# lmdu/pyfastx

Measured on AMD Instinct MI355X. Metric: FASTA index build + 1M random 100bp subseq fetches, 3 Gbp plain FASTA per GPU (throughput of the whole step, stream resident in HBM), higher is better.
Workload: dtype u8; 1 GPU; configs[1]: synthetic 3.0 Gbp hg38-shaped plain FASTA per GPU (200 contigs, 60-col LF, soft-masked, N runs), index build + 1000000 random 100 bp intervals (50% '-' strand); parallelism=one GPU, the whole stream resident in its HBM

## Files before the change

pyfastx_amd/csrc/fx_spanscan.hpp:

```cpp
#pragma once
#include "fx_kernels.hpp"

namespace fx {

#ifndef FX_GRAN
#define FX_GRAN 4096
#endif
constexpr int GRAN = FX_GRAN;
constexpr int GR_ROWS = GRAN / (64 * CHUNK);
constexpr int SPAN_GRANS = 65536 / GRAN;
constexpr int SPAN = GRAN * SPAN_GRANS;
constexpr uint32_t SP_NONE = 0xFFFFFFFFu;

struct GranOut { uint32_t n, h, first, last, v1, c1, v2, c2, ovf; };
struct __attribute__((aligned(16))) GranPk { uint32_t nh, fl, d1, d2; };
__device__ __forceinline__ GranPk gran_pack(const GranOut &o) {
    GranPk p;
    p.nh = o.n | (o.h << 16); p.fl = (o.first & 0xFFFFu) | (o.last << 16);
    p.d1 = o.v1 | (o.c1 << 16); p.d2 = o.v2 | (o.c2 << 16) | (o.ovf << 31);
    return p;
}
__device__ __forceinline__ GranOut gran_unpack(const GranPk &p) {
    GranOut o;
    o.n = p.nh & 0xFFFFu; o.h = p.nh >> 16;
// ... 196 lines not shown
#define FX_SCAN_GPW 1
#endif
constexpr int SCAN_GPW = FX_SCAN_GPW;
template <int MODE>
__global__ __launch_bounds__(1024) void k_span_scan(const uint8_t *__restrict__ data, int64_t n, int prev_byte,
                                                   int is_last, int64_t g_end, GranPk *__restrict__ out, GranList hgl) {
    __shared__ uint32_t hl_n, hl_done, hl_g[16 * SCAN_GPW];
    if (MODE == 0) {
        if (threadIdx.x == 0) { hl_n = 0; hl_done = 0; }
        __syncthreads();
    }
    const int64_t g0 = (((int64_t)blockIdx.x * blockDim.x + threadIdx.x) >> 6) * SCAN_GPW;
    uint4 v[SCAN_GPW][GR_ROWS];
#pragma unroll
    for (int k = 0; k < SCAN_GPW; ++k) if (g0 + k < g_end) granule_load<true>(v[k], data, n, is_last, g0 + k);
    uint32_t L = 0, hmask = 0;
#pragma unroll
    for (int k = 0; k < SCAN_GPW; ++k)
        if (g0 + k < g_end && granule_body<MODE>(v[k], data, prev_byte, g0 + k, out, L)) hmask |= 1u << k;
    if (MODE == 0 && lane_id() == 0) {
#pragma unroll
        for (int k = 0; k < SCAN_GPW; ++k) if ((hmask >> k) & 1u) hl_g[atomicAdd(&hl_n, 1u)] = (uint32_t)(g0 + k);
        __threadfence_block();
        if (atomicAdd(&hl_done, 1u) == (blockDim.x >> 6) - 1) {
            const uint32_t cnt = hl_n;
            if (cnt) {
                const uint32_t base = atomicAdd(hgl.count, cnt);
                for (uint32_t k = 0; k < cnt; ++k) hgl.g[base + k] = hl_g[k];
            }
        }
    }
}

constexpr int CHUNK_GRANS = 1024;
struct ChunkTot { long long n, h, last, pad; };
struct Totals {
    long long n_nl, n_hdr, last_nl, seq_len, pad0, pad1, pad2, pad3;
};

__device__ __forceinline__ long long shfl_up64(long long v, int d) {
    const int lo = __shfl_up((int)(v & 0xFFFFFFFFll), d, 64), hi = __shfl_up((int)(v >> 32), d, 64);
    return ((long long)hi << 32) | (unsigned int)lo;
}
__device__ __forceinline__ long long shfl64(long long v, int l) {
    const int lo = __shfl((int)(v & 0xFFFFFFFFll), l, 64), hi = __shfl((int)(v >> 32), l, 64);
    return ((long long)hi << 32) | (unsigned int)lo;
}
struct Tri { long long n, h, last; };
__device__ __forceinline__ Tri tri_join(const Tri &a, const Tri &b) { return Tri{a.n + b.n, a.h + b.h, a.last > b.last ? a.last : b.last}; }
__device__ __forceinline__ Tri tri_wave_incl(Tri v) {
    const int l = lane_id();
#pragma unroll
    for (int d = 1; d < 64; d <<= 1) {
        const Tri t{shfl_up64(v.n, d), shfl_up64(v.h, d), shfl_up64(v.last, d)};
        if (l >= d) v = tri_join(t, v);
    }
    return v;
}
__device__ __forceinline__ Tri tri_block_incl(Tri v, Tri *lds, Tri *total) {
    const int w = threadIdx.x >> 6, l = lane_id(), nw = (blockDim.x + 63) >> 6;
    const Tri inc = tri_wave_incl(v);
    __syncthreads();
    if (l == 63) lds[w] = inc;
    __syncthreads();
    Tri base{0, 0, -1}, tot{0, 0, -1};
    for (int i = 0; i < nw; ++i) { const Tri s = lds[i]; if (i < w) base = tri_join(base, s); tot = tri_join(tot, s); }
    *total = tot;
    return tri_join(base, inc);
}
__device__ __forceinline__ Tri gran_tri(const GranPk *__restrict__ go, int64_t g, int64_t ngran, int64_t gbase) {
    if (g >= ngran) return Tri{0, 0, -1};
    const GranOut o = gran_unpack(go[g]);
    return Tri{(long long)o.n, (long long)o.h, o.n ? gbase + g * (long long)GRAN + o.last : -1};
}

template <int MODE, int CG>
__global__ __launch_bounds__(CG) void k_gran_reduce(const uint8_t *__restrict__ data, int64_t n, int prev_byte,
                                                   int is_last, GranList hgl, GranPk *__restrict__ go,
                                                   int64_t ngran, int64_t gbase, ChunkTot *__restrict__ ct) {
    __shared__ Tri lds[CG / 64];
    if (blockIdx.x == gridDim.x - 1) {
        if (threadIdx.x < 64) {
            uint32_t L = 0;
            const uint32_t h_w = granule<false, MODE>(data, n, prev_byte, is_last, ngran - 1, go, L);
            if (MODE == 0 && h_w && threadIdx.x == 0) hgl.g[atomicAdd(hgl.count, 1u)] = (uint32_t)(ngran - 1);
        }
        __threadfence_block();
        __syncthreads();
    }
    Tri tot;
    tri_block_incl(gran_tri(go, (int64_t)blockIdx.x * CG + threadIdx.x, ngran, gbase), lds, &tot);
    if (threadIdx.x == 0) ct[blockIdx.x] = ChunkTot{tot.n, tot.h, tot.last, 0};
}

struct Tri32 { uint32_t n, h; int32_t last; };
__device__ __forceinline__ Tri32 tri32_block_incl(Tri32 v, uint32_t (*lds)[16], Tri32 *total) {
    const int w = threadIdx.x >> 6, l = lane_id(), nw = (blockDim.x + 63) >> 6;
#pragma unroll
    for (int d = 1; d < 64; d <<= 1) {
        const uint32_t a = __shfl_up(v.n, d, 64), b = __shfl_up(v.h, d, 64);
        const int32_t c = __shfl_up(v.last, d, 64);
        if (l >= d) { v.n += a; v.h += b; v.last = c > v.last ? c : v.last; }
    }
    __syncthreads();
    if (l == 63) { lds[0][w] = v.n; lds[1][w] = v.h; lds[2][w] = (uint32_t)v.last; }
    __syncthreads();
    Tri32 base{0, 0, -1}, tot{0, 0, -1};
    for (int i = 0; i < nw; ++i) {
        const uint32_t a = lds[0][i], b = lds[1][i];
        const int32_t c = (int32_t)lds[2][i];
        if (i < w) { base.n += a; base.h += b; base.last = c > base.last ? c : base.last; }
        tot.n += a; tot.h += b; tot.last = c > tot.last ? c : tot.last;
    }
    *total = tot;
    return Tri32{base.n + v.n, base.h + v.h, base.last > v.last ? base.last : v.last};
}

template <int CG>
__global__ __launch_bounds__(CG) void k_gran_prefix(const GranPk *__restrict__ go, int64_t ngran, int64_t gbase,
                                                            const ChunkTot *__restrict__ ct, Totals *__restrict__ tot,
                                                            int64_t *__restrict__ nl_prefix, int64_t *__restrict__ hdr_prefix,
                                                            int64_t *__restrict__ prevnl) {
    __shared__ Tri lds[CG / 64];
    __shared__ uint32_t lds32[3][16];
    Tri b{0, 0, -1};
    for (int64_t c = threadIdx.x; c < (int64_t)blockIdx.x; c += CG) { const ChunkTot t = ct[c]; b = tri_join(b, Tri{t.n, t.h, t.last}); }
    Tri base{0, 0, -1};
    if (blockIdx.x) tri_block_incl(b, lds, &base);
    const int64_t g = (int64_t)blockIdx.x * CG + threadIdx.x;
    Tri32 v{0, 0, -1};
    if (g < ngran) {
        const GranOut o = gran_unpack(go[g]);
        v = Tri32{o.n, o.h, o.n ? (int32_t)(threadIdx.x * GRAN + o.last) : -1};
    }
    Tri32 total;
    const Tri32 inc = tri32_block_incl(v, lds32, &total);
    const int64_t cstart = gbase + (int64_t)blockIdx.x * CG * GRAN;
    if (g < ngran) {
        nl_prefix[g] = base.n + (inc.n - v.n);
        hdr_prefix[g] = base.h + (inc.h - v.h);
        int32_t pm = __shfl_up(inc.last, 1, 64);
        if (lane_id() == 0) { pm = -1; for (int i = 0; i < (int)(threadIdx.x >> 6); ++i) { const int32_t c = (int32_t)lds32[2][i]; pm = c > pm ? c : pm; } }
        prevnl[g] = pm >= 0 ? cstart + pm : base.last;
    }
    if (blockIdx.x == gridDim.x - 1 && threadIdx.x == 0) {
        const int64_t tn = base.n + total.n, th = base.h + total.h, tl = total.last >= 0 ? cstart + total.last : base.last;
        nl_prefix[ngran] = tn; hdr_prefix[ngran] = th; prevnl[ngran] = tl;
        tot->n_nl = tn; tot->n_hdr = th; tot->last_nl = tl;
    }
}

struct ScanCtx {
    const uint8_t *data; int64_t n, gbase, ngran;
    const GranPk *go;
    const int64_t *nl_prefix, *hdr_prefix, *prevnl;
};

__device__ __forceinline__ int64_t next_nl(const ScanCtx &c, int64_t x) {
    const int64_t y = x + 1 - c.gbase;
    if (y > c.n) return -1;
    const int64_t g = y / GRAN;
    if (g < c.ngran) {
        const GranOut o = gran_unpack(c.go[g]);
        const int64_t gs = g * (int64_t)GRAN;
        if (o.n && gs + o.last >= y) {
            if (gs + o.first >= y) return c.gbase + gs + o.first;
            for (int64_t p = y & ~(int64_t)(CHUNK - 1); p < gs + GRAN; p += CHUNK) {
                const uint4 v = load16(c.data, p, c.n);
                uint32_t m = eq_mask16(v, 0x0A0A0A0Au);
                if (p < y) m &= 0xFFFFu << (y - p);
                if (m) return c.gbase + p + (__ffs(m) - 1);
                if (p + CHUNK > c.n) break;
            }
            return c.gbase + gs + o.last;
        }
    }
    const int64_t key = c.gbase + (g + 1) * (int64_t)GRAN;
    int64_t lo = g + 1, hi = c.ngran;
// ... 285 lines not shown
            return;
        }
    }
    irr.g[atomicAdd(irr.count, 1u)] = (uint32_t)g;
}

__global__ __launch_bounds__(BLOCK) void k_gran_exact(ScanCtx x, RecView rv, int64_t cap, GranList irr, int is_last, int prev_byte) {
    const int lane = lane_id();
    const int64_t wave = ((int64_t)blockIdx.x * blockDim.x + threadIdx.x) >> 6;
    const int64_t nwaves = ((int64_t)gridDim.x * blockDim.x) >> 6;
    const int64_t cnt = *irr.count;
    int64_t i = wave, g = i < cnt ? irr.g[i] : 0;
    uint4 v[GR_ROWS];
    if (i < cnt) {
#pragma unroll
        for (int j = 0; j < GR_ROWS; ++j) v[j] = load16(x.data, g * (int64_t)GRAN + j * 1024 + lane * CHUNK, x.n);
    }
    for (; i < cnt; i += nwaves) {
        const int64_t gc = g, hb = x.hdr_prefix[gc];
        int64_t he = x.hdr_prefix[gc + 1];
        if (he > cap) he = cap;
        ExactMasks mk;
        exact_masks(x, v, is_last, prev_byte, gc, he > hb, mk);
        if (i + nwaves < cnt) {
            g = irr.g[i + nwaves];
#pragma unroll
            for (int j = 0; j < GR_ROWS; ++j) v[j] = load16(x.data, g * (int64_t)GRAN + j * 1024 + lane * CHUNK, x.n);
        }
        exact_rows(x, rv, cap, gc, hb, mk);
    }
}

__global__ __launch_bounds__(BLOCK) void k_fasta_finalize2(int64_t cap, FastaCols c, Totals *__restrict__ tot,
                                                          const uint8_t *__restrict__ data, int64_t n_bytes, int64_t gbase) {
    const int64_t *__restrict__ hdr = c.hoff, *__restrict__ hdr_line = c.hdr_line;
    const int64_t k = (int64_t)blockIdx.x * BLOCK + threadIdx.x;
    const int64_t n_hdr = tot->n_hdr < cap ? tot->n_hdr : cap;
    int64_t s = 0;
    if (k < n_hdr) {
        if (c.dlen[k] >= 0) {
            int64_t hn, Ln;
            if (k + 1 < n_hdr) { hn = hdr[k + 1]; Ln = hdr_line[k + 1]; }
            else               { hn = tot->last_nl + 1; Ln = tot->n_nl; }
            const int64_t nseq = Ln - hdr_line[k] - 1;
            const int64_t blen = hn - c.boff[k];
            s = blen - (int64_t)c.elen[k] * nseq;
            c.blen[k] = blen; c.slen[k] = s;
            const int norm = c.bad[k] > 1 ? 0 : 1;
            c.norm[k] = norm;
            int reg = line_regular(data, n_bytes, gbase, c.boff[k], blen, s, nseq > 0 ? c.llen[k] : 0, c.elen[k], norm);
            if (reg < 0) reg = c.bad[k] == 0;
            c.reg[k] = reg;
        } else { c.blen[k] = 0; c.slen[k] = 0; c.norm[k] = 1; c.reg[k] = 0; }
    }
    __shared__ unsigned long long blk;
    if (threadIdx.x == 0) blk = 0;
    __syncthreads();
    s = wave_sum64(s);
    if (lane_id() == 0 && s) atomicAdd(&blk, (unsigned long long)s);
    __syncthreads();
    if (threadIdx.x == 0 && blk) atomicAdd((unsigned long long *)&tot->seq_len, blk);
}

__global__ __launch_bounds__(BLOCK) void k_line_regular(const uint8_t *__restrict__ data, int64_t n_bytes, int64_t gbase, int64_t n,
                                                       const int64_t *__restrict__ boff, const int64_t *__restrict__ blen,
                                                       const int64_t *__restrict__ slen, const int64_t *__restrict__ llen,
                                                       const int32_t *__restrict__ elen, const int32_t *__restrict__ norm,
                                                       int32_t *__restrict__ reg) {
    const int64_t k = (int64_t)blockIdx.x * BLOCK + threadIdx.x;
    if (k < n) reg[k] = line_regular(data, n_bytes, gbase, boff[k], blen[k], slen[k], llen[k], elen[k], norm[k]) > 0 ? 1 : 0;
}

__device__ __forceinline__ int64_t prev_nl_wave(const ScanCtx &x, int64_t p) {
    const int64_t y = (p - x.gbase < x.n) ? p - x.gbase : x.n;
    if (y <= 0) return -1;
    const int64_t g = (y - 1) / GRAN;
    const int64_t a = g * (int64_t)GRAN + lane_id() * 64;
    unsigned long long m = 0;
#pragma unroll
    for (int i = 0; i < 4; ++i)
        if (a + i * CHUNK < y) m |= (unsigned long long)eq_mask16(load16(x.data, a + i * CHUNK, x.n), 0x0A0A0A0Au) << (16 * i);
    if (y - a < 64) m &= (y - a <= 0) ? 0ull : (~0ull >> (64 - (y - a)));
    const unsigned long long b = __ballot(m != 0);
    if (!b) return x.prevnl[g];
    const int l = 63 - __clzll(b);
    const int hi = __shfl((int)(m >> 32), l, 64), lo = __shfl((int)(m & 0xFFFFFFFFull), l, 64);
    const unsigned long long ml = ((unsigned long long)(unsigned int)hi << 32) | (unsigned int)lo;
    return x.gbase + g * (int64_t)GRAN + l * 64 + (63 - __clzll(ml));
}

constexpr int SUMM_BLOCK = 1024;
__device__ __forceinline__ DiffSet diffset_shfl_xor(const DiffSet &d, int m) {
    return DiffSet{(uint32_t)__shfl_xor((int)d.v1, m, 64), (uint32_t)__shfl_xor((int)d.c1, m, 64), (uint32_t)__shfl_xor((int)d.v2, m, 64),
                   (uint32_t)__shfl_xor((int)d.c2, m, 64), (uint32_t)__shfl_xor((int)d.ovf, m, 64)};
// ... 210 lines not shown
```

pyfastx_amd/csrc/fxgpu.hip:

```cpp
#include <hip/hip_runtime.h>
#include <zlib.h>
#include <fcntl.h>
#include <pthread.h>
#include <sched.h>
#include <sys/mman.h>
#include <sys/stat.h>
#include <unistd.h>

#include <algorithm>
#include <atomic>
#include <chrono>
#include <functional>
#include <map>
#include <memory>
#include <cstdarg>
#include <cstdio>
#include <cstdlib>
#include <cstring>
#include <mutex>
#include <string>
#include <thread>
#include <vector>

#include "../../include/fxgpu.h"
// ... 223 lines not shown
        if (count <= 0) return FX_OK;
        dev = device;
        stream = st;
        p = (T *)g_scratch.get(device, (size_t)count * sizeof(T), &cap_bytes);
        if (!p) return fail(FX_ENOMEM, "hipMalloc(%lld B) failed", (long long)(count * sizeof(T)));
        return FX_OK;
    }
    void release() {
        if (p) { (void)hipStreamSynchronize(stream); g_scratch.put(dev, p, cap_bytes); }
        p = nullptr; cap_bytes = 0;
    }
    ~ScratchBuf() { release(); }
};

static void crc_tables(CrcTables *T) {
    for (uint32_t i = 0; i < 256; ++i) { uint32_t c = i; for (int k = 0; k < 8; ++k) c = (c & 1) ? 0xEDB88320u ^ (c >> 1) : c >> 1; T->crc[0][i] = c; }
    for (int j = 1; j < 4; ++j)
        for (uint32_t i = 0; i < 256; ++i) T->crc[j][i] = (T->crc[j - 1][i] >> 8) ^ T->crc[0][T->crc[j - 1][i] & 0xFFu];
    uint32_t a[32], b[32];
    a[0] = 0xEDB88320u;
    for (int n = 1; n < 32; ++n) a[n] = 1u << (n - 1);
    auto times = [](const uint32_t *mat, uint32_t vec) { uint32_t s = 0; for (int i = 0; vec; vec >>= 1, ++i) if (vec & 1) s ^= mat[i]; return s; };
    for (int r = 0; r < 3; ++r) { for (int n = 0; n < 32; ++n) b[n] = times(a, a[n]); memcpy(a, b, sizeof a); }
    for (int j = 0; j < 17; ++j) {
        memcpy(T->pow2[j], a, sizeof a);
        for (int n = 0; n < 32; ++n) b[n] = times(a, a[n]);
        memcpy(a, b, sizeof a);
    }
    for (int k = 0; k < CRC_NSH; ++k)
        for (int byte = 0; byte < 4; ++byte)
            for (uint32_t v = 0; v < 256; ++v) T->sh[k][byte][v] = times(T->pow2[CRC_SH0 + k], v << (8 * byte));
}

enum KernelId { K_SPAN_SCAN = 0, K_GRAN_REDUCE, K_GRAN_PREFIX, K_HDR_REC, K_GRAN_LINES, K_GRAN_EXACT, K_FASTA_FINALIZE, K_FETCH,
                K_FASTA_COMP, K_FASTA_COMP_EDGE, K_FASTA_COMP_SMALL, K_FASTQ_LINES, K_FASTQ_ROWS, K_FASTQ_EMIT, K_FASTQ_STATS, K_FASTQ_COMP, K_FASTQ_FETCH, K_BGZF_INFLATE, K_BGZF_COPY, K_BGZF_CRC, K_SCAN_COMP, K_COMP_ATTRIBUTE, K_BGZF_SERIAL, K_FETCH_REST, K_KQ_LINES, K_KQ_PREFIX, K_KQ_WALK, K_KQ_GATHER, K_NKERN };
static const char *const kKernelNames[K_NKERN] = {
    "k_span_scan", "k_gran_reduce", "k_gran_prefix", "k_hdr_rec", "k_gran_lines", "k_gran_exact", "k_fasta_finalize", "k_fetch",
    "k_fasta_comp", "k_fasta_comp_edge", "k_fasta_comp_small", "k_fastq_lines", "k_fastq_rows", "k_fastq_emit", "k_fastq_stats", "k_fastq_comp", "k_fastq_fetch", "k_bgzf_decode", "k_bgzf_copy", "k_bgzf_crc", "k_scan_comp", "k_comp_attribute", "k_bgzf_decode_serial", "k_fetch_rest", "k_kq_lines", "k_kq_prefix", "k_kq_walk", "k_kq_gather"};

struct Prof {
    bool on = false;
    uint32_t mask = ~0u;
    struct Span { int id; hipEvent_t a, b; };
    std::vector<Span> pending;
    std::vector<hipEvent_t> pool;
    double ms[K_NKERN] = {0};
    int64_t cnt[K_NKERN] = {0};
    hipEvent_t get() {
        if (!pool.empty()) { hipEvent_t e = pool.back(); pool.pop_back(); return e; }
        hipEvent_t e = nullptr;
        (void)hipEventCreate(&e);
        return e;
    }
    bool hit = false;
    void begin(int id, hipStream_t s) {
        hit = on && ((mask >> id) & 1u);
        if (!hit) return;
        Span sp{id, get(), get()};
        (void)hipEventRecord(sp.a, s);
        pending.push_back(sp);
    }
    void end(hipStream_t s) { if (hit) (void)hipEventRecord(pending.back().b, s); }
    void drain() {
        for (auto &sp : pending) {
            float t = 0.f;
            if (hipEventElapsedTime(&t, sp.a, sp.b) == hipSuccess) { ms[sp.id] += t; cnt[sp.id]++; }
            pool.push_back(sp.a); pool.push_back(sp.b);
        }
        pending.clear();
    }
    ~Prof() { drain(); for (auto e : pool) (void)hipEventDestroy(e); }
};
#define FX_LAUNCH(h, id, kern, grid, block, ...)                                  \
    do {                                                                          \
        (h)->prof.begin(id, (h)->stream);                                         \
        hipLaunchKernelGGL(kern, grid, block, 0, (h)->stream, __VA_ARGS__);       \
        (h)->prof.end((h)->stream);                                               \
    } while (0)

struct StageAsync;
static void stage_drop(fx_handle *h);
struct fx_handle {
    int device = 0;
    hipStream_t stream = nullptr;
    StageAsync *stage = nullptr;
    int stage_fd = -1;
    hipStream_t stream2 = nullptr;
    uint8_t *d_data = nullptr;
    uint8_t *d_alloc = nullptr;
    size_t blob_cap = 0;
    bool owns = false;
    int64_t n = 0;
    bool gz = false;
    int64_t base = 0;
    int prev_byte = '\n';
    bool is_last = true;
    int64_t n_nl = 0;
    bool scanned = false;
    int64_t ngran = 0;
    DevBuf<GranPk> gran;
    DevBuf<uint32_t> hdr_grans, irr_grans;
    DevBuf<ChunkTot> chunks;
    DevBuf<unsigned long long> ctl;
    Totals *pin_tot = nullptr;
    struct OneBox { int64_t off, blen, skip, take, dst_off, out_len; } *one_box = nullptr;
    uint8_t *one_out = nullptr;
    Mailbox *mb = nullptr;
    hipStream_t mb_stream = nullptr;
    unsigned long long mb_seq = 0;
    bool mb_running = false, mb_off = false;
    DevBuf<uint32_t> nm_table;
    DevBuf<int64_t> nm_off;
    uint64_t nm_mask = 0;
    int nm_kind = -1;
    DevBuf<int64_t> nl_prefix, hdr_prefix, prevnl;
    DevBuf<int64_t> hdr, fa_boff, fa_blen, fa_slen, fa_llen, fa_hdr_line;
    DevBuf<int32_t> fa_elen, fa_norm, fa_dlen, fa_name_len, fa_reg;
    DevBuf<uint32_t> fa_bad;
    int64_t n_hdr = 0, fa_seqlen = 0;
    bool fasta_built = false;
    bool build_pending = false;
    int pending_full_name = 0;
    DevBuf<uint32_t> comp_runs;
    int comp_gpw = 0;
    bool comp_runs_valid = false;
    DevBuf<int64_t> fq_name_off, fq_rlen, fq_soff, fq_qoff;
    DevBuf<int32_t> fq_name_len, fq_dlen, fq_qlen;
    DevBuf<FastqAcc> fq_acc;
    DevBuf<FqRun> fq_runs;
    DevBuf<FastqAcc> fq_acc_build;
    DevBuf<uint32_t> fq_rej;
    int64_t fq_comp_runs = 0, fq_comp_rejected = 0;
    bool fq_comp_valid = false;
    int64_t fq_comp_base[5] = {0, 0, 0, 0, 0};
    int fq_comp_minqs = 104, fq_comp_maxqs = 33;
// ... 1530 lines not shown
    ScanCtx x;
    x.data = h->d_data; x.n = h->n; x.gbase = h->base; x.ngran = h->ngran;
    x.go = h->gran.p; x.nl_prefix = h->nl_prefix.p; x.hdr_prefix = h->hdr_prefix.p; x.prevnl = h->prevnl.p;
    return x;
}
static FastaCols fasta_cols(fx_handle *h) {
    FastaCols c;
    c.hoff = h->hdr.p; c.boff = h->fa_boff.p; c.blen = h->fa_blen.p; c.slen = h->fa_slen.p; c.llen = h->fa_llen.p;
    c.hdr_line = h->fa_hdr_line.p; c.elen = h->fa_elen.p; c.dlen = h->fa_dlen.p; c.name_len = h->fa_name_len.p;
    c.norm = h->fa_norm.p; c.bad = h->fa_bad.p; c.reg = h->fa_reg.p;
    return c;
}
static int alloc_fasta_table(fx_handle *h, int64_t cap) {
    int rc;
    if ((rc = h->hdr.alloc(cap)) || (rc = h->fa_hdr_line.alloc(cap)) || (rc = h->fa_boff.alloc(cap)) ||
        (rc = h->fa_blen.alloc(cap)) || (rc = h->fa_slen.alloc(cap)) || (rc = h->fa_llen.alloc(cap)) ||
        (rc = h->fa_elen.alloc(cap)) || (rc = h->fa_norm.alloc(cap)) || (rc = h->fa_dlen.alloc(cap)) ||
        (rc = h->fa_name_len.alloc(cap)) || (rc = h->fa_bad.alloc(cap)) || (rc = h->fa_reg.alloc(cap)))
        return rc;
    return FX_OK;
}

static Totals *ctl_totals(fx_handle *h) { return (Totals *)h->ctl.p; }
static uint32_t *ctl_counter(fx_handle *h, int i) { return (uint32_t *)(h->ctl.p + 8 + i); }

static int comp_run_granules(int64_t ngran) {
    return ngran >= 65536 ? 4 * COMP_DEPTH : ngran >= 16384 ? 2 * COMP_DEPTH : COMP_DEPTH;
}

template <int MODE>
static int granule_pass(fx_handle *h, bool fq_lines = false, bool with_comp = false) {
    int rc;
    const int64_t nfull = h->n / GRAN, ngran = nfull + 1;
    const bool small = ngran <= (2ll << 20);
    const int64_t cg = small ? 256 : 1024, nchunks = (ngran + cg - 1) / cg;
    h->ngran = ngran;
    if ((rc = h->gran.alloc(ngran)) || (rc = h->hdr_grans.alloc(ngran)) || (MODE == 0 && (rc = h->irr_grans.alloc(ngran))) ||
        (rc = h->chunks.alloc(nchunks)) ||
        (rc = h->ctl.alloc(64)) || (rc = h->nl_prefix.alloc(ngran + 1)) || (rc = h->hdr_prefix.alloc(ngran + 1)) ||
        (rc = h->prevnl.alloc(ngran + 1)))
        return rc;
    if (!h->pin_tot) HIPCHK(hipHostMalloc((void **)&h->pin_tot, sizeof(Totals), hipHostMallocDefault));
    HIPCHK(hipMemsetAsync(h->ctl.p, 0, 64 * sizeof(unsigned long long), h->stream));
    GranList hgl{h->hdr_grans.p, ctl_counter(h, 0)};
    const int SCAN_WG = 512;
    if (nfull > 0 && MODE == 1 && fq_lines) {
        if ((rc = h->fq_lines.alloc((nfull + FQR_G - 1) / FQR_G * FQR_G * FQL_CAP))) return rc;
        if (with_comp) {
            const int64_t nruns = (nfull + FQLC_G - 1) / FQLC_G;
            if ((rc = h->fq_runs.alloc(nruns)) || (rc = h->fq_acc_build.alloc(1)) || (rc = h->fq_rej.alloc(nruns + 1))) return rc;
            static const int64_t grid_cap = [] { const char *e = getenv("FX_FQ_FUSED_GRID"); return e && atoll(e) > 0 ? atoll(e) : 6144ll; }();
            static const int force_crlf = [] { const char *e = getenv("FX_FQ_CRLF"); return e ? atoi(e) : -1; }();
            if (force_crlf >= 0 ? force_crlf != 0 : h->fq_crlf)
                FX_LAUNCH(h, K_FASTQ_LINES, k_fastq_lines_comp<true>, dim3((unsigned)std::min<int64_t>(nblocks(nruns, BLOCK / 64), grid_cap)), dim3(BLOCK), h->d_data,
                          h->n, h->prev_byte, nfull, h->gran.p, h->fq_lines.p, hgl, h->fq_runs.p, nruns);
            else
                FX_LAUNCH(h, K_FASTQ_LINES, k_fastq_lines_comp<false>, dim3((unsigned)std::min<int64_t>(nblocks(nruns, BLOCK / 64), grid_cap)), dim3(BLOCK), h->d_data,
                          h->n, h->prev_byte, nfull, h->gran.p, h->fq_lines.p, hgl, h->fq_runs.p, nruns);
        } else
        FX_LAUNCH(h, K_FASTQ_LINES, k_fastq_lines, dim3(nblocks(nfull, (BLOCK / 64) * FQL_G)), dim3(BLOCK), h->d_data, h->n, h->prev_byte, nfull,
                  h->gran.p, h->fq_lines.p, hgl);
    } else if (nfull > 0 && MODE == 0 && with_comp) {
        const int gpw = comp_run_granules(ngran);
        const int64_t runs = (ngran + gpw - 1) / gpw;
        if ((rc = h->comp_runs.alloc(runs * RUN_WORDS))) return rc;
        HIPCHK(hipMemsetAsync(h->comp_runs.p, 0, (size_t)runs * RUN_WORDS * 4, h->stream));
        FX_LAUNCH(h, K_SCAN_COMP, k_scan_comp, dim3(nblocks(runs, COMP_WPB)), dim3(COMP_WPB * 64), h->d_data, h->n, h->prev_byte,
                  (int)h->is_last, nfull, h->gran.p, hgl, gpw, h->comp_runs.p);
        h->comp_gpw = gpw;
        h->comp_runs_valid = true;
    } else if (nfull > 0)
        FX_LAUNCH(h, K_SPAN_SCAN, (k_span_scan<MODE>), dim3(nblocks((nfull + SCAN_GPW - 1) / SCAN_GPW * 64, SCAN_WG)), dim3(SCAN_WG), h->d_data, h->n,
                  h->prev_byte, (int)h->is_last, nfull, h->gran.p, hgl);
    if (small) {
        FX_LAUNCH(h, K_GRAN_REDUCE, (k_gran_reduce<MODE, 256>), dim3((unsigned)nchunks), dim3(256), h->d_data, h->n, h->prev_byte,
                  (int)h->is_last, hgl, h->gran.p, ngran, h->base, h->chunks.p);
        FX_LAUNCH(h, K_GRAN_PREFIX, (k_gran_prefix<256>), dim3((unsigned)nchunks), dim3(256), h->gran.p, ngran, h->base,
                  h->chunks.p, ctl_totals(h), h->nl_prefix.p, h->hdr_prefix.p, h->prevnl.p);
    } else {
        FX_LAUNCH(h, K_GRAN_REDUCE, (k_gran_reduce<MODE, 1024>), dim3((unsigned)nchunks), dim3(1024), h->d_data, h->n, h->prev_byte,
                  (int)h->is_last, hgl, h->gran.p, ngran, h->base, h->chunks.p);
        FX_LAUNCH(h, K_GRAN_PREFIX, (k_gran_prefix<1024>), dim3((unsigned)nchunks), dim3(1024), h->gran.p, ngran, h->base,
                  h->chunks.p, ctl_totals(h), h->nl_prefix.p, h->hdr_prefix.p, h->prevnl.p);
    }
    if (MODE == 1 && fq_lines && with_comp && nfull > 0) {
        FastqAcc init;
        memset(&init, 0, sizeof init);
        init.minqs = 104; init.maxqs = 33;
        HIPCHK(hipMemcpyAsync(h->fq_acc_build.p, &init, sizeof init, hipMemcpyHostToDevice, h->stream));
        const int64_t nruns = (nfull + FQLC_G - 1) / FQLC_G;
        HIPCHK(hipMemsetAsync(h->fq_rej.p, 0, 4, h->stream));
        FX_LAUNCH(h, K_FASTQ_COMP, k_fastq_comp_reduce, dim3((unsigned)std::min<int64_t>(nblocks(nruns, BLOCK), 1024)), dim3(BLOCK), (const FqRun *)h->fq_runs.p,
                  nruns, (const int64_t *)h->nl_prefix.p, (int64_t)0, h->d_data, h->n, nfull, h->fq_acc_build.p, h->fq_rej.p);
    }
    HIPCHK(hipGetLastError());
    return FX_OK;
}

static int enqueue_records(fx_handle *h, int full_name) {
    const ScanCtx x = scan_ctx(h);
    const int64_t cap = h->hdr.cap, ngran = h->ngran;
    const FastaCols c = fasta_cols(h);
    const RecView rv{h->fa_boff.p, h->fa_llen.p, h->fa_dlen.p, h->fa_bad.p, h->hdr.p};
    const GranList hgl{h->hdr_grans.p, ctl_counter(h, 0)}, irr{h->irr_grans.p, ctl_counter(h, 1)};
    FX_LAUNCH(h, K_HDR_REC, k_hdr_rec, dim3(2048), dim3(BLOCK), x, h->prev_byte, (int)h->is_last, full_name, hgl, c, cap);
    FX_LAUNCH(h, K_GRAN_LINES, k_gran_lines, dim3(nblocks(ngran, BLOCK)), dim3(BLOCK), x, rv, cap, irr);
    FX_LAUNCH(h, K_GRAN_EXACT, k_gran_exact, dim3(2048), dim3(BLOCK), x, rv, cap, irr, (int)h->is_last, h->prev_byte);
    FX_LAUNCH(h, K_FASTA_FINALIZE, k_fasta_finalize2, dim3(nblocks(cap, BLOCK)), dim3(BLOCK), cap, c, ctl_totals(h), h->d_data, h->n, h->base);
    HIPCHK(hipGetLastError());
    HIPCHK(hipMemcpyAsync(h->pin_tot, ctl_totals(h), sizeof(Totals), hipMemcpyDeviceToHost, h->stream));
    return FX_OK;
}

extern "C" int fx_fasta_build_begin(fx_handle *h, int full_name) {
    if (!h) return fail(FX_EINVAL, "null handle");
    int rc = use_device(h);
    if (rc) return rc;
    if (h->n <= 0) return fail(FX_EFORMAT, "empty input");
    h->scanned = false;
    h->nm_kind = -1;
    const bool with_comp = (full_name & 2) != 0;
    full_name &= 1;
    h->comp_runs_valid = false;
    if ((rc = granule_pass<0>(h, false, with_comp))) return rc;
    if (h->hdr.cap < 4096 && (rc = alloc_fasta_table(h, 4096))) return rc;
    if ((rc = enqueue_records(h, full_name))) return rc;
    h->build_pending = true;
    h->pending_full_name = full_name;
    h->fasta_built = true;
    return FX_OK;
}

static int finish_build(fx_handle *h) {
    if (!h->build_pending) return FX_OK;
    int rc = use_device(h);
    if (rc) return rc;
    Totals tot;
    for (;;) {
        HIPCHK(hipStreamSynchronize(h->stream));
        tot = *h->pin_tot;
        if (tot.n_hdr <= h->hdr.cap) break;
        if ((rc = alloc_fasta_table(h, tot.n_hdr + tot.n_hdr / 16 + 16))) return rc;
        HIPCHK(hipMemsetAsync(&ctl_totals(h)->seq_len, 0, 8, h->stream));
        HIPCHK(hipMemsetAsync(ctl_counter(h, 1), 0, 4, h->stream));
        if ((rc = enqueue_records(h, h->pending_full_name))) return rc;
    }
    h->build_pending = false;
    h->n_hdr = tot.n_hdr;
    h->n_nl = tot.n_nl;
    h->fa_seqlen = tot.seq_len;
    if (tot.n_hdr <= 0 && h->base == 0 && h->is_last) { h->fasta_built = false; return fail(FX_EFORMAT, "no FASTA header line ('>') found"); }
    return FX_OK;
}

extern "C" int fx_fasta_build_end(fx_handle *h, fx_fasta_summary *out) {
    if (!h) return fail(FX_EINVAL, "null handle");
    if (!h->fasta_built) return fail(FX_ESTATE, "fx_fasta_build_begin has not run");
    int rc = finish_build(h);
    if (rc) return rc;
    if (out) { out->n_seq = h->n_hdr; out->seq_len = h->fa_seqlen; out->n_lines = h->n_nl; out->n_bytes = h->n; }
    return FX_OK;
}

extern "C" int fx_fasta_build(fx_handle *h, int full_name, fx_fasta_summary *out) {
    int rc = fx_fasta_build_begin(h, full_name);
    if (rc) return rc;
    return fx_fasta_build_end(h, out);
}

extern "C" int fx_fasta_set_table(fx_handle *h, int64_t n, const int64_t *boff, const int64_t *blen, const int64_t *slen,
                                  const int64_t *llen, const int32_t *elen, const int32_t *norm) {
    if (!h || n < 0 || (n > 0 && (!boff || !blen || !slen || !llen || !elen || !norm))) return fail(FX_EINVAL, "bad argument");
    int rc = use_device(h);
// ... 186 lines not shown
    lc.lap(2);
    if (with_comp) {
        const int64_t nfull = h->n / GRAN, nruns = (nfull + FQLC_G - 1) / FQLC_G;
        h->fq_comp_runs = nruns;
        h->fq_comp_rejected = n_rej;
        static const int64_t rej_div = [] { const char *e = getenv("FX_FQ_RECOUNT_DIV"); return e && atoll(e) > 0 ? atoll(e) : 8ll; }();
        if (built.qfix == 0 && n_rej > 0) {
            if ((int64_t)n_rej <= std::max<int64_t>(64, nruns / rej_div)) {
                const int64_t pieces = (int64_t)n_rej * (FQLC_G / FS_GPW);
                FX_LAUNCH(h, K_FASTQ_COMP, k_fastq_comp_stream, dim3((unsigned)std::min<int64_t>(nblocks(pieces, BLOCK / 64), 2048)), dim3(BLOCK), h->d_data, h->n, nfull,
                          (const int64_t *)h->nl_prefix.p, (int64_t)0, h->fq_acc_build.p, (const uint32_t *)(h->fq_rej.p + 1), (int64_t)n_rej, (int)FQLC_G);
                HIPCHK(hipGetLastError());
                HIPCHK(hipMemcpyAsync(&built, h->fq_acc_build.p, sizeof built, hipMemcpyDeviceToHost, h->stream));
                HIPCHK(hipStreamSynchronize(h->stream));
            } else {
                built.qfix = 1;
                h->fq_comp_rejected = -1;
            }
        }
    }
    if (with_comp && built.qfix == 0) {
        h->fq_comp_valid = true;
        h->fq_comp_base[0] = (int64_t)built.a; h->fq_comp_base[1] = (int64_t)built.c; h->fq_comp_base[2] = (int64_t)built.g;
        h->fq_comp_base[3] = (int64_t)built.t; h->fq_comp_base[4] = (int64_t)built.n;
        h->fq_comp_minqs = built.minqs; h->fq_comp_maxqs = built.maxqs;
    }
    h->fq_by_lines = by_lines;
    if (by_lines) {
        const uint32_t tail = (uint32_t)(h->ngran - 1);
        HIPCHK(hipMemcpyAsync(h->hdr_grans.p + n_over, &tail, sizeof tail, hipMemcpyHostToDevice, h->stream));
        HIPCHK(hipStreamSynchronize(h->stream));
        h->fq_nlist = (int64_t)n_over + 1;
    }
    h->n_nl = h->pin_tot->n_nl;
    h->fq_c2 = host[2];
    h->scanned = true;
    if (n_nl_core) *n_nl_core = host[0];
    if (last_nl_core) *last_nl_core = host[1];
    return FX_OK;
}

struct FqPlan { FqOwn own; int64_t n_reads, n_seq; };
static int fastq_plan(fx_handle *h, int64_t loff, int64_t prev_nl, FqPlan *pl) {
    const int64_t N = h->n_nl;
    const int64_t k0 = (loff + 3) / 4;
    const int64_t k_first = k0 + ((loff % 4 == 0 && prev_nl + 1 < h->base) ? 1 : 0);
    const int64_t core_len = h->n - h->halo;
    const int64_t k_end = core_len > 0 ? (loff + h->fq_c2) / 4 + 1 : k_first;
    const int64_t complete = (loff + N) / 4;
    const int64_t nrows = std::max<int64_t>(k_end - k_first, 0);
    pl->n_reads = std::max<int64_t>(std::min(k_end, complete) - k_first, 0);
    pl->n_seq = loff + N >= 2 ? std::max<int64_t>(std::min(k_end, (loff + N - 2) / 4 + 1) - k_first, 0) : 0;
    if (!h->is_last && k_end > complete)
        return fail(FX_ERANGE, "a FASTQ record that starts in this shard runs past its %lld-byte halo", (long long)h->halo);
    pl->own = FqOwn{loff, prev_nl, k_first, nrows};
    return FX_OK;
}
static int fastq_alloc(fx_handle *h, int64_t cap) {
    int rc;
    cap = std::max<int64_t>(cap, 1);
    if ((rc = h->fq_name_off.alloc(cap)) || (rc = h->fq_rlen.alloc(cap)) || (rc = h->fq_soff.alloc(cap)) ||
        (rc = h->fq_qoff.alloc(cap)) || (rc = h->fq_name_len.alloc(cap)) || (rc = h->fq_dlen.alloc(cap)) ||
        (rc = h->fq_qlen.alloc(cap)) || (rc = h->fq_acc.alloc(1)))
        return rc;
    return FX_OK;
}
// ... 2405 lines not shown
```

Before: 4906 Gbp/s.

## Replace two-kernel granule reduce/prefix with single-pass decoupled look-back scan

Merges the granule reduce kernel and the prefix kernel into one chained-scan kernel. It uses dynamic ticketing, per-chunk aggregate and inclusive flags with epochs, and a wave-parallel look-back. Each thread handles 16 granules, which cuts the second pass over granule data and one launch. The finalize kernel now writes totals straight to pinned host memory from the last block, replacing a separate async memcpy. The spin-waits add a risk of stalls and a timeout error path.

```diff
diff --git a/pyfastx_amd/csrc/fx_spanscan.hpp b/pyfastx_amd/csrc/fx_spanscan.hpp
--- a/pyfastx_amd/csrc/fx_spanscan.hpp
+++ b/pyfastx_amd/csrc/fx_spanscan.hpp
@@ -252,10 +252,13 @@
     }
 }
 
-constexpr int CHUNK_GRANS = 1024;
-struct ChunkTot { long long n, h, last, pad; };
+constexpr int CHAIN_WG = 512;
+inline int chain_gpt(int64_t) { return 16; }
+constexpr uint32_t CHAIN_AGG = 1, CHAIN_INCL = 2;
+constexpr int CHAIN_SPIN_MAX = 1 << 20;
+struct ChunkDesc { long long an, ah, alast, in, ih, ilast; uint32_t flag, pad; uint64_t pad2; };
 struct Totals {
-    long long n_nl, n_hdr, last_nl, seq_len, pad0, pad1, pad2, pad3;
+    long long n_nl, n_hdr, last_nl, seq_len, err, pad1, pad2, pad3;
 };
 
 __device__ __forceinline__ long long shfl_up64(long long v, int d) {
@@ -268,53 +271,18 @@
 }
 struct Tri { long long n, h, last; };
 __device__ __forceinline__ Tri tri_join(const Tri &a, const Tri &b) { return Tri{a.n + b.n, a.h + b.h, a.last > b.last ? a.last : b.last}; }
-__device__ __forceinline__ Tri tri_wave_incl(Tri v) {
-    const int l = lane_id();
-#pragma unroll
-    for (int d = 1; d < 64; d <<= 1) {
-        const Tri t{shfl_up64(v.n, d), shfl_up64(v.h, d), shfl_up64(v.last, d)};
-        if (l >= d) v = tri_join(t, v);
-    }
+__device__ __forceinline__ long long shfl_xor64(long long v, int m) {
+    const int lo = __shfl_xor((int)(v & 0xFFFFFFFFll), m, 64), hi = __shfl_xor((int)(v >> 32), m, 64);
+    return ((long long)hi << 32) | (unsigned int)lo;
+}
+__device__ __forceinline__ Tri tri_wave_all(Tri v) {
+#pragma unroll
+    for (int m = 1; m < 64; m <<= 1) v = tri_join(v, Tri{shfl_xor64(v.n, m), shfl_xor64(v.h, m), shfl_xor64(v.last, m)});
     return v;
 }
-__device__ __forceinline__ Tri tri_block_incl(Tri v, Tri *lds, Tri *total) {
-    const int w = threadIdx.x >> 6, l = lane_id(), nw = (blockDim.x + 63) >> 6;
-    const Tri inc = tri_wave_incl(v);
-    __syncthreads();
-    if (l == 63) lds[w] = inc;
-    __syncthreads();
-    Tri base{0, 0, -1}, tot{0, 0, -1};
-    for (int i = 0; i < nw; ++i) { const Tri s = lds[i]; if (i < w) base = tri_join(base, s); tot = tri_join(tot, s); }
-    *total = tot;
-    return tri_join(base, inc);
-}
-__device__ __forceinline__ Tri gran_tri(const GranPk *__restrict__ go, int64_t g, int64_t ngran, int64_t gbase) {
-    if (g >= ngran) return Tri{0, 0, -1};
-    const GranOut o = gran_unpack(go[g]);
-    return Tri{(long long)o.n, (long long)o.h, o.n ? gbase + g * (long long)GRAN + o.last : -1};
-}
-
-template <int MODE, int CG>
-__global__ __launch_bounds__(CG) void k_gran_reduce(const uint8_t *__restrict__ data, int64_t n, int prev_byte,
-                                                   int is_last, GranList hgl, GranPk *__restrict__ go,
-                                                   int64_t ngran, int64_t gbase, ChunkTot *__restrict__ ct) {
-    __shared__ Tri lds[CG / 64];
-    if (blockIdx.x == gridDim.x - 1) {
-        if (threadIdx.x < 64) {
-            uint32_t L = 0;
-            const uint32_t h_w = granule<false, MODE>(data, n, prev_byte, is_last, ngran - 1, go, L);
-            if (MODE == 0 && h_w && threadIdx.x == 0) hgl.g[atomicAdd(hgl.count, 1u)] = (uint32_t)(ngran - 1);
-        }
-        __threadfence_block();
-        __syncthreads();
-    }
-    Tri tot;
-    tri_block_incl(gran_tri(go, (int64_t)blockIdx.x * CG + threadIdx.x, ngran, gbase), lds, &tot);
-    if (threadIdx.x == 0) ct[blockIdx.x] = ChunkTot{tot.n, tot.h, tot.last, 0};
-}
 
 struct Tri32 { uint32_t n, h; int32_t last; };
-__device__ __forceinline__ Tri32 tri32_block_incl(Tri32 v, uint32_t (*lds)[16], Tri32 *total) {
+__device__ __forceinline__ Tri32 tri32_block_excl(Tri32 v, uint32_t (*lds)[16], Tri32 *total) {
     const int w = threadIdx.x >> 6, l = lane_id(), nw = (blockDim.x + 63) >> 6;
 #pragma unroll
     for (int d = 1; d < 64; d <<= 1) {
@@ -322,7 +290,8 @@
         const int32_t c = __shfl_up(v.last, d, 64);
         if (l >= d) { v.n += a; v.h += b; v.last = c > v.last ? c : v.last; }
     }
-    __syncthreads();
+    Tri32 ex{__shfl_up(v.n, 1, 64), __shfl_up(v.h, 1, 64), __shfl_up(v.last, 1, 64)};
+    if (l == 0) ex = Tri32{0, 0, -1};
     if (l == 63) { lds[0][w] = v.n; lds[1][w] = v.h; lds[2][w] = (uint32_t)v.last; }
     __syncthreads();
     Tri32 base{0, 0, -1}, tot{0, 0, -1};
@@ -333,37 +302,147 @@
         tot.n += a; tot.h += b; tot.last = c > tot.last ? c : tot.last;
     }
     *total = tot;
-    return Tri32{base.n + v.n, base.h + v.h, base.last > v.last ? base.last : v.last};
-}
-
-template <int CG>
-__global__ __launch_bounds__(CG) void k_gran_prefix(const GranPk *__restrict__ go, int64_t ngran, int64_t gbase,
-                                                            const ChunkTot *__restrict__ ct, Totals *__restrict__ tot,
-                                                            int64_t *__restrict__ nl_prefix, int64_t *__restrict__ hdr_prefix,
-                                                            int64_t *__restrict__ prevnl) {
-    __shared__ Tri lds[CG / 64];
+    return Tri32{base.n + ex.n, base.h + ex.h, base.last > ex.last ? base.last : ex.last};
+}
+
+__device__ __forceinline__ uint32_t chain_wait(const uint32_t *flag, uint32_t epoch) {
+    for (int k = 0; k < CHAIN_SPIN_MAX; ++k) {
+        const uint32_t f = __hip_atomic_load(flag, __ATOMIC_RELAXED, __HIP_MEMORY_SCOPE_AGENT);
+        if ((f >> 2) == epoch && (f & 3u)) return f & 3u;
+        __builtin_amdgcn_s_sleep(1);
+    }
+    return 0;
+}
+
+__device__ __forceinline__ Tri chain_lookback(const ChunkDesc *d, int64_t c, uint32_t epoch, bool *bad) {
+    const int lane = lane_id();
+    Tri acc{0, 0, -1};
+    for (int64_t top = c - 1; top >= 0; top -= 64) {
+        const int64_t j = top - lane;
+        const uint32_t st = j >= 0 ? chain_wait(&d[j].flag, epoch) : CHAIN_INCL;
+        __builtin_amdgcn_fence(__ATOMIC_ACQUIRE, "agent");
+        const unsigned long long stop = __ballot(st != CHAIN_AGG);
+        const int k = stop ? __ffsll(stop) - 1 : 63;
+        Tri v{0, 0, -1};
+        if (lane <= k && j >= 0) {
+            if (st == CHAIN_INCL) v = Tri{d[j].in, d[j].ih, d[j].ilast};
+            else if (st == CHAIN_AGG) v = Tri{d[j].an, d[j].ah, d[j].alast};
+        }
+        acc = tri_join(acc, tri_wave_all(v));
+        if (__ballot(st == 0)) { *bad = true; break; }
+        if (stop) break;
+    }
+    return acc;
+}
+
+__device__ __forceinline__ void chain_publish(ChunkDesc *d, const Tri &v, bool incl, uint32_t epoch) {
+    if (incl) { d->in = v.n; d->ih = v.h; d->ilast = v.last; }
+    else      { d->an = v.n; d->ah = v.h; d->alast = v.last; }
+    __hip_atomic_store(&d->flag, epoch << 2 | (incl ? CHAIN_INCL : CHAIN_AGG), __ATOMIC_RELEASE, __HIP_MEMORY_SCOPE_AGENT);
+}
+
+template <int MODE, int GPT>
+__global__ __launch_bounds__(CHAIN_WG) void k_gran_chain(const uint8_t *__restrict__ data, int64_t n, int prev_byte, int is_last,
+                                                         GranList hgl, GranPk *__restrict__ go, int64_t ngran, int64_t gbase,
+                                                         ChunkDesc *__restrict__ desc, int64_t nchunks, uint32_t epoch,
+                                                         uint32_t *__restrict__ ticket, Totals *__restrict__ tot,
+                                                         int64_t *__restrict__ nl_prefix, int64_t *__restrict__ hdr_prefix,
+                                                         int64_t *__restrict__ prevnl) {
+    constexpr int CG = CHAIN_WG * GPT;
     __shared__ uint32_t lds32[3][16];
-    Tri b{0, 0, -1};
-    for (int64_t c = threadIdx.x; c < (int64_t)blockIdx.x; c += CG) { const ChunkTot t = ct[c]; b = tri_join(b, Tri{t.n, t.h, t.last}); }
-    Tri base{0, 0, -1};
-    if (blockIdx.x) tri_block_incl(b, lds, &base);
-    const int64_t g = (int64_t)blockIdx.x * CG + threadIdx.x;
-    Tri32 v{0, 0, -1};
-    if (g < ngran) {
-        const GranOut o = gran_unpack(go[g]);
-        v = Tri32{o.n, o.h, o.n ? (int32_t)(threadIdx.x * GRAN + o.last) : -1};
-    }
-    Tri32 total;
-    const Tri32 inc = tri32_block_incl(v, lds32, &total);
-    const int64_t cstart = gbase + (int64_t)blockIdx.x * CG * GRAN;
-    if (g < ngran) {
-        nl_prefix[g] = base.n + (inc.n - v.n);
-        hdr_prefix[g] = base.h + (inc.h - v.h);
-        int32_t pm = __shfl_up(inc.last, 1, 64);
-        if (lane_id() == 0) { pm = -1; for (int i = 0; i < (int)(threadIdx.x >> 6); ++i) { const int32_t c = (int32_t)lds32[2][i]; pm = c > pm ? c : pm; } }
-        prevnl[g] = pm >= 0 ? cstart + pm : base.last;
-    }
-    if (blockIdx.x == gridDim.x - 1 && threadIdx.x == 0) {
+    __shared__ int64_t s_c;
+    __shared__ Tri s_base;
+    if (threadIdx.x == 0) s_c = (int64_t)atomicAdd(ticket, 1u) - 1;
+    __syncthreads();
+    const int64_t c = s_c;
+    if (c < 0) {
+        if (threadIdx.x < 64) {
+            uint32_t L = 0;
+            const uint32_t h_w = granule<false, MODE>(data, n, prev_byte, is_last, ngran - 1, go, L);
+            if (threadIdx.x == 0) {
+                if (MODE == 0 && h_w) hgl.g[atomicAdd(hgl.count, 1u)] = (uint32_t)(ngran - 1);
+                __hip_atomic_store(&desc[nchunks].flag, epoch << 2 | CHAIN_INCL, __ATOMIC_RELEASE, __HIP_MEMORY_SCOPE_AGENT);
+            }
+        }
+        return;
+    }
+    bool bad = false;
+    const int lane = lane_id(), w = threadIdx.x >> 6, nw = CHAIN_WG / 64;
+    const int64_t cg0 = c * CG;
+    const int wl0 = w * 64 * GPT;
+    if (c == nchunks - 1) {
+        const int rt = (int)(ngran - 1 - cg0);
+        if (rt >= wl0 && rt < wl0 + 64 * GPT && (rt & 63) == lane) {
+            if (!chain_wait(&desc[nchunks].flag, epoch)) bad = true;
+            __builtin_amdgcn_fence(__ATOMIC_ACQUIRE, "agent");
+        }
+    }
+    GranPk pk[GPT];
+#pragma unroll
+    for (int k = 0; k < GPT; ++k) {
+        const int64_t g = cg0 + wl0 + k * 64 + lane;
+        if (g < ngran) pk[k] = go[g];
+    }
+    uint32_t en[GPT], eh[GPT];
+    int32_t el[GPT];
+    Tri32 carry{0, 0, -1};
+#pragma unroll
+    for (int k = 0; k < GPT; ++k) {
+        const int r = wl0 + k * 64 + lane;
+        Tri32 v{0, 0, -1};
+        if (cg0 + r < ngran) {
+            const GranOut o = gran_unpack(pk[k]);
+            v = Tri32{o.n, o.h, o.n ? (int32_t)(r * GRAN + o.last) : -1};
+        }
+#pragma unroll
+        for (int d = 1; d < 64; d <<= 1) {
+            const uint32_t a = __shfl_up(v.n, d, 64), b = __shfl_up(v.h, d, 64);
+            const int32_t e = __shfl_up(v.last, d, 64);
+            if (lane >= d) { v.n += a; v.h += b; v.last = e > v.last ? e : v.last; }
+        }
+        uint32_t xn = __shfl_up(v.n, 1, 64), xh = __shfl_up(v.h, 1, 64);
+        int32_t xl = __shfl_up(v.last, 1, 64);
+        if (lane == 0) { xn = 0; xh = 0; xl = -1; }
+        en[k] = carry.n + xn; eh[k] = carry.h + xh; el[k] = xl > carry.last ? xl : carry.last;
+        const int32_t tl = __shfl(v.last, 63, 64);
+        carry.n += __shfl(v.n, 63, 64); carry.h += __shfl(v.h, 63, 64); carry.last = tl > carry.last ? tl : carry.last;
+    }
+    if (lane == 0) { lds32[0][w] = carry.n; lds32[1][w] = carry.h; lds32[2][w] = (uint32_t)carry.last; }
+    __syncthreads();
+    Tri32 woff{0, 0, -1}, total{0, 0, -1};
+    for (int i = 0; i < nw; ++i) {
+        const uint32_t a = lds32[0][i], b = lds32[1][i];
+        const int32_t e = (int32_t)lds32[2][i];
+        if (i < w) { woff.n += a; woff.h += b; woff.last = e > woff.last ? e : woff.last; }
+        total.n += a; total.h += b; total.last = e > total.last ? e : total.last;
+    }
+    const int64_t cstart = gbase + c * CG * (int64_t)GRAN;
+    if (threadIdx.x < 64) {
+        const Tri agg{(long long)total.n, (long long)total.h, total.last >= 0 ? cstart + total.last : -1};
+        Tri base{0, 0, -1};
+        if (c == 0) {
+            if (threadIdx.x == 0) chain_publish(&desc[0], agg, true, epoch);
+        } else {
+            if (threadIdx.x == 0) chain_publish(&desc[c], agg, false, epoch);
+            base = chain_lookback(desc, c, epoch, &bad);
+            if (threadIdx.x == 0) chain_publish(&desc[c], tri_join(base, agg), true, epoch);
+        }
+        if (threadIdx.x == 0) s_base = base;
+    }
+    if (bad) atomicOr((unsigned long long *)&tot->err, 1ull);
+    __syncthreads();
+    const Tri base = s_base;
+#pragma unroll
+    for (int k = 0; k < GPT; ++k) {
+        const int64_t g = cg0 + wl0 + k * 64 + lane;
+        if (g < ngran) {
+            const int32_t l = el[k] > woff.last ? el[k] : woff.last;
+            nl_prefix[g] = base.n + woff.n + en[k];
+            hdr_prefix[g] = base.h + woff.h + eh[k];
+            prevnl[g] = l >= 0 ? cstart + l : base.last;
+        }
+    }
+    if (c == nchunks - 1 && threadIdx.x == 0) {
         const int64_t tn = base.n + total.n, th = base.h + total.h, tl = total.last >= 0 ? cstart + total.last : base.last;
         nl_prefix[ngran] = tn; hdr_prefix[ngran] = th; prevnl[ngran] = tl;
         tot->n_nl = tn; tot->n_hdr = th; tot->last_nl = tl;
@@ -715,7 +794,8 @@
 }
 
 __global__ __launch_bounds__(BLOCK) void k_fasta_finalize2(int64_t cap, FastaCols c, Totals *__restrict__ tot,
-                                                          const uint8_t *__restrict__ data, int64_t n_bytes, int64_t gbase) {
+                                                          const uint8_t *__restrict__ data, int64_t n_bytes, int64_t gbase,
+                                                          Totals *__restrict__ host_tot, uint32_t *__restrict__ done) {
     const int64_t *__restrict__ hdr = c.hoff, *__restrict__ hdr_line = c.hdr_line;
     const int64_t k = (int64_t)blockIdx.x * BLOCK + threadIdx.x;
     const int64_t n_hdr = tot->n_hdr < cap ? tot->n_hdr : cap;
@@ -742,7 +822,15 @@
     s = wave_sum64(s);
     if (lane_id() == 0 && s) atomicAdd(&blk, (unsigned long long)s);
     __syncthreads();
-    if (threadIdx.x == 0 && blk) atomicAdd((unsigned long long *)&tot->seq_len, blk);
+    if (threadIdx.x == 0) {
+        if (blk) atomicAdd((unsigned long long *)&tot->seq_len, blk);
+        if (__hip_atomic_fetch_add(done, 1u, __ATOMIC_ACQ_REL, __HIP_MEMORY_SCOPE_AGENT) == gridDim.x - 1) {
+            *done = 0;
+            long long *src = (long long *)tot, *dst = (long long *)host_tot;
+            for (int i = 0; i < (int)(sizeof(Totals) / 8); ++i) dst[i] = __hip_atomic_load(&src[i], __ATOMIC_RELAXED, __HIP_MEMORY_SCOPE_AGENT);
+            __threadfence_system();
+        }
+    }
 }
 
 __global__ __launch_bounds__(BLOCK) void k_line_regular(const uint8_t *__restrict__ data, int64_t n_bytes, int64_t gbase, int64_t n,
diff --git a/pyfastx_amd/csrc/fxgpu.hip b/pyfastx_amd/csrc/fxgpu.hip
--- a/pyfastx_amd/csrc/fxgpu.hip
+++ b/pyfastx_amd/csrc/fxgpu.hip
@@ -279,10 +279,10 @@
             for (uint32_t v = 0; v < 256; ++v) T->sh[k][byte][v] = times(T->pow2[CRC_SH0 + k], v << (8 * byte));
 }
 
-enum KernelId { K_SPAN_SCAN = 0, K_GRAN_REDUCE, K_GRAN_PREFIX, K_HDR_REC, K_GRAN_LINES, K_GRAN_EXACT, K_FASTA_FINALIZE, K_FETCH,
+enum KernelId { K_SPAN_SCAN = 0, K_GRAN_CHAIN, K_HDR_REC, K_GRAN_LINES, K_GRAN_EXACT, K_FASTA_FINALIZE, K_FETCH,
                 K_FASTA_COMP, K_FASTA_COMP_EDGE, K_FASTA_COMP_SMALL, K_FASTQ_LINES, K_FASTQ_ROWS, K_FASTQ_EMIT, K_FASTQ_STATS, K_FASTQ_COMP, K_FASTQ_FETCH, K_BGZF_INFLATE, K_BGZF_COPY, K_BGZF_CRC, K_SCAN_COMP, K_COMP_ATTRIBUTE, K_BGZF_SERIAL, K_FETCH_REST, K_KQ_LINES, K_KQ_PREFIX, K_KQ_WALK, K_KQ_GATHER, K_NKERN };
 static const char *const kKernelNames[K_NKERN] = {
-    "k_span_scan", "k_gran_reduce", "k_gran_prefix", "k_hdr_rec", "k_gran_lines", "k_gran_exact", "k_fasta_finalize", "k_fetch",
+    "k_span_scan", "k_gran_chain", "k_hdr_rec", "k_gran_lines", "k_gran_exact", "k_fasta_finalize", "k_fetch",
     "k_fasta_comp", "k_fasta_comp_edge", "k_fasta_comp_small", "k_fastq_lines", "k_fastq_rows", "k_fastq_emit", "k_fastq_stats", "k_fastq_comp", "k_fastq_fetch", "k_bgzf_decode", "k_bgzf_copy", "k_bgzf_crc", "k_scan_comp", "k_comp_attribute", "k_bgzf_decode_serial", "k_fetch_rest", "k_kq_lines", "k_kq_prefix", "k_kq_walk", "k_kq_gather"};
 
 struct Prof {
@@ -347,7 +347,8 @@
     int64_t ngran = 0;
     DevBuf<GranPk> gran;
     DevBuf<uint32_t> hdr_grans, irr_grans;
-    DevBuf<ChunkTot> chunks;
+    DevBuf<ChunkDesc> chunks;
+    uint32_t chain_epoch = 0;
     DevBuf<unsigned long long> ctl;
     Totals *pin_tot = nullptr;
     struct OneBox { int64_t off, blen, skip, take, dst_off, out_len; } *one_box = nullptr;
@@ -1944,15 +1945,18 @@
 static int granule_pass(fx_handle *h, bool fq_lines = false, bool with_comp = false) {
     int rc;
     const int64_t nfull = h->n / GRAN, ngran = nfull + 1;
-    const bool small = ngran <= (2ll << 20);
-    const int64_t cg = small ? 256 : 1024, nchunks = (ngran + cg - 1) / cg;
+    const int gpt = chain_gpt(ngran);
+    const int64_t nchunks = (ngran + (int64_t)CHAIN_WG * gpt - 1) / ((int64_t)CHAIN_WG * gpt);
+    const bool fresh = h->chunks.cap < nchunks + 1;
     h->ngran = ngran;
     if ((rc = h->gran.alloc(ngran)) || (rc = h->hdr_grans.alloc(ngran)) || (MODE == 0 && (rc = h->irr_grans.alloc(ngran))) ||
-        (rc = h->chunks.alloc(nchunks)) ||
+        (rc = h->chunks.alloc(nchunks + 1)) ||
         (rc = h->ctl.alloc(64)) || (rc = h->nl_prefix.alloc(ngran + 1)) || (rc = h->hdr_prefix.alloc(ngran + 1)) ||
         (rc = h->prevnl.alloc(ngran + 1)))
         return rc;
     if (!h->pin_tot) HIPCHK(hipHostMalloc((void **)&h->pin_tot, sizeof(Totals), hipHostMallocDefault));
+    if (fresh) HIPCHK(hipMemsetAsync(h->chunks.p, 0, (size_t)h->chunks.cap * sizeof(ChunkDesc), h->stream));
+    h->chain_epoch = h->chain_epoch % ((1u << 30) - 1) + 1;
     HIPCHK(hipMemsetAsync(h->ctl.p, 0, 64 * sizeof(unsigned long long), h->stream));
     GranList hgl{h->hdr_grans.p, ctl_counter(h, 0)};
     const int SCAN_WG = 512;
@@ -1984,17 +1988,15 @@
     } else if (nfull > 0)
         FX_LAUNCH(h, K_SPAN_SCAN, (k_span_scan<MODE>), dim3(nblocks((nfull + SCAN_GPW - 1) / SCAN_GPW * 64, SCAN_WG)), dim3(SCAN_WG), h->d_data, h->n,
                   h->prev_byte, (int)h->is_last, nfull, h->gran.p, hgl);
-    if (small) {
-        FX_LAUNCH(h, K_GRAN_REDUCE, (k_gran_reduce<MODE, 256>), dim3((unsigned)nchunks), dim3(256), h->d_data, h->n, h->prev_byte,
-                  (int)h->is_last, hgl, h->gran.p, ngran, h->base, h->chunks.p);
-        FX_LAUNCH(h, K_GRAN_PREFIX, (k_gran_prefix<256>), dim3((unsigned)nchunks), dim3(256), h->gran.p, ngran, h->base,
-                  h->chunks.p, ctl_totals(h), h->nl_prefix.p, h->hdr_prefix.p, h->prevnl.p);
-    } else {
-        FX_LAUNCH(h, K_GRAN_REDUCE, (k_gran_reduce<MODE, 1024>), dim3((unsigned)nchunks), dim3(1024), h->d_data, h->n, h->prev_byte,
-                  (int)h->is_last, hgl, h->gran.p, ngran, h->base, h->chunks.p);
-        FX_LAUNCH(h, K_GRAN_PREFIX, (k_gran_prefix<1024>), dim3((unsigned)nchunks), dim3(1024), h->gran.p, ngran, h->base,
-                  h->chunks.p, ctl_totals(h), h->nl_prefix.p, h->hdr_prefix.p, h->prevnl.p);
-    }
+    uint32_t *ticket = (uint32_t *)(h->ctl.p + 10);
+    if (gpt == 4)
+        FX_LAUNCH(h, K_GRAN_CHAIN, (k_gran_chain<MODE, 4>), dim3((unsigned)(nchunks + 1)), dim3(CHAIN_WG), h->d_data, h->n, h->prev_byte,
+                  (int)h->is_last, hgl, h->gran.p, ngran, h->base, h->chunks.p, nchunks, h->chain_epoch, ticket, ctl_totals(h),
+                  h->nl_prefix.p, h->hdr_prefix.p, h->prevnl.p);
+    else
+        FX_LAUNCH(h, K_GRAN_CHAIN, (k_gran_chain<MODE, 16>), dim3((unsigned)(nchunks + 1)), dim3(CHAIN_WG), h->d_data, h->n, h->prev_byte,
+                  (int)h->is_last, hgl, h->gran.p, ngran, h->base, h->chunks.p, nchunks, h->chain_epoch, ticket, ctl_totals(h),
+                  h->nl_prefix.p, h->hdr_prefix.p, h->prevnl.p);
     if (MODE == 1 && fq_lines && with_comp && nfull > 0) {
         FastqAcc init;
         memset(&init, 0, sizeof init);
@@ -2018,9 +2020,9 @@
     FX_LAUNCH(h, K_HDR_REC, k_hdr_rec, dim3(2048), dim3(BLOCK), x, h->prev_byte, (int)h->is_last, full_name, hgl, c, cap);
     FX_LAUNCH(h, K_GRAN_LINES, k_gran_lines, dim3(nblocks(ngran, BLOCK)), dim3(BLOCK), x, rv, cap, irr);
     FX_LAUNCH(h, K_GRAN_EXACT, k_gran_exact, dim3(2048), dim3(BLOCK), x, rv, cap, irr, (int)h->is_last, h->prev_byte);
-    FX_LAUNCH(h, K_FASTA_FINALIZE, k_fasta_finalize2, dim3(nblocks(cap, BLOCK)), dim3(BLOCK), cap, c, ctl_totals(h), h->d_data, h->n, h->base);
+    FX_LAUNCH(h, K_FASTA_FINALIZE, k_fasta_finalize2, dim3(nblocks(cap, BLOCK)), dim3(BLOCK), cap, c, ctl_totals(h), h->d_data, h->n, h->base,
+              h->pin_tot, (uint32_t *)(h->ctl.p + 12));
     HIPCHK(hipGetLastError());
-    HIPCHK(hipMemcpyAsync(h->pin_tot, ctl_totals(h), sizeof(Totals), hipMemcpyDeviceToHost, h->stream));
     return FX_OK;
 }
 
@@ -2051,6 +2053,7 @@
     for (;;) {
         HIPCHK(hipStreamSynchronize(h->stream));
         tot = *h->pin_tot;
+        if (tot.err) { h->build_pending = false; h->fasta_built = false; return fail(FX_EDEVICE, "granule prefixes: a look-back flag never came"); }
         if (tot.n_hdr <= h->hdr.cap) break;
         if ((rc = alloc_fasta_table(h, tot.n_hdr + tot.n_hdr / 16 + 16))) return rc;
         HIPCHK(hipMemsetAsync(&ctl_totals(h)->seq_len, 0, 8, h->stream));
@@ -2303,6 +2306,7 @@
         HIPCHK(hipStreamSynchronize(h->stream));
         h->fq_nlist = (int64_t)n_over + 1;
     }
+    if (h->pin_tot->err) return fail(FX_EDEVICE, "granule prefixes: a look-back flag never came");
     h->n_nl = h->pin_tot->n_nl;
     h->fq_c2 = host[2];
     h->scanned = true;
```

Measured after the change: 4873 Gbp/s (median of 3 runs). Within noise of the previous version (-0.7%).
